# facebookresearch/wmar

Hardware: AMD Instinct MI355X
Metric: watermarked images/sec at 256x256 (16x16 tok), batch 64; detector p-value delta vs ref (higher is better)
Workload: dtype f32; 1 GPU; Taming cin_transformer (48L x 1536d x 24h, V=16384) + VQGAN f16/16384, 256x256, batch 64 per GPU, greenlist watermark delta=2 gamma=0.25 h=1 (linear/stratifiedrand), T=1 top-k 250 top-p 0.92; sample -> decode -> re-encode -> detect; random-init weights; batch_per_gpu=64, decode_loop=hipGraph replay, backend=nccl

## Files before the change

wmar_amd/csrc/decoder_kernels.h:

```cpp
#pragma once
#include <cstdint>

#include "sampler.h"
#include "bx_split.h"

namespace wmar {

using f32x16 = __attribute__((ext_vector_type(16))) float;
using f32x4 = __attribute__((ext_vector_type(4))) float;

__device__ __forceinline__ float4 ld_nt(const float4* p) {
    f32x4 v = __builtin_nontemporal_load((const f32x4*)p);
    return make_float4(v.x, v.y, v.z, v.w);
}

__device__ __forceinline__ void st_out(float4* p, const float4 v) {
#ifndef WMAR_PLAIN_STORES
    const f32x4 q = {v.x, v.y, v.z, v.w};
    asm volatile("global_store_dwordx4 %0, %1, off sc1\n\ts_nop 1" :: "v"(p), "v"(q) : "memory");
#else
    *p = v;
#endif
}
using f32x2 = __attribute__((ext_vector_type(2))) float;
// ... 677 lines not shown

constexpr int QX_CK = 4;
#ifndef QX_ABL
#define QX_ABL 0
#endif
#define WMAR_QX_SYNC() if (!(QX_ABL & 2)) __syncthreads();
#ifndef QX_SPLIT
#define QX_SPLIT 2
#endif

struct QkvxArgs {
    const float4* Wp;
    const float4* x_in;
    float4* x_out;
    const float4* slabs;
    long long slab_stride;
    int n_hi;
    const float* bias;
    double* stats;
    float4* out;
    long long out_stride;
    int KB, NT, S, cap;
    int nkeep;
    unsigned long long* trace;
    unsigned long long* trace_chunks;
};

template <int MTW, int S_IN>
__global__ __launch_bounds__(512) void k_qkvx(QkvxArgs a) {
    __shared__ __attribute__((aligned(16))) float4 xs[2][QX_CK][MTW][64];
    __shared__ double red[4][MTW][64][2];
    const int lane = threadIdx.x & 63;
    const int w = __builtin_amdgcn_readfirstlane(threadIdx.x >> 6);
    const int half = lane >> 5;
    const int G = a.NT >> 2;
    const int j = (int)(blockIdx.x & 7) * a.cap + (int)(blockIdx.x >> 3);
    if (j >= G * a.S) return;
    const int s = j / G, g = j - s * G;
    const int kb0 = (int)((unsigned)s * (unsigned)a.KB / (unsigned)a.S);
    const int kb1 = (int)((unsigned)(s + 1) * (unsigned)a.KB / (unsigned)a.S);
    const int nkb = kb1 - kb0, nch = (nkb + QX_CK - 1) / QX_CK;
    const bool keeper = g == 0;

    if (w >= 4) {
        const int sw = w - 4;
        double sum[MTW], sq[MTW];
// ... 191 lines not shown
static int launch_qkvx(const QkvxArgs& q, int MT, int S_in, hipStream_t st) {
    if (MT == 1) return launch_qkvx_mt<1>(q, S_in, st);
    if (MT == 2) return launch_qkvx_mt<2>(q, S_in, st);
    set_error("qkvx: %d row tiles unsupported", MT);
    return WMAR_EINVAL;
}

static __global__ void k_pack_bx(const float* __restrict__ W, const float* __restrict__ gamma, float4* __restrict__ Wq, int N, int K,
                                      int tile_off) {
    const long long idx = (long long)blockIdx.x * blockDim.x + threadIdx.x;
    const int KU = K / 16;
    if (idx >= (long long)(N / 32) * KU * 128) return;
    const int lane = (int)(idx & 63), hf = (int)((idx >> 6) & 1);
    const long long r = idx >> 7;
    const int ku = (int)(r % KU), tile = (int)(r / KU);
    const int k = ku * 16 + 8 * (lane >> 5) + 4 * hf;
    const float* p = W + (long long)(tile * 32 + (lane & 31)) * K + k;
    float4 v = make_float4(p[0], p[1], p[2], p[3]);
    if (gamma) { v.x *= gamma[k]; v.y *= gamma[k + 1]; v.z *= gamma[k + 2]; v.w *= gamma[k + 3]; }
    Wq[idx + (long long)tile_off * KU * 128] = v;
}

constexpr int QX_TR_STRIDE = 36;
template <int S_IN>
__global__ __launch_bounds__(512) void k_qkvx_bx(QkvxArgs a) {
    constexpr int MTW = 2;
    __shared__ __attribute__((aligned(16))) u32x4 xq[2][2][MTW][3][64];
    __shared__ __attribute__((aligned(16))) float tr_s[4][32 * QX_TR_STRIDE];
    __shared__ double red[4][MTW][64][2];
    const int lane = threadIdx.x & 63;
    const int w = __builtin_amdgcn_readfirstlane(threadIdx.x >> 6);
    const int half = lane >> 5;
    const int G = a.NT >> 2;
    const int j = (int)(blockIdx.x & 7) * a.cap + (int)(blockIdx.x >> 3);
    if (j >= G * a.S) return;
    const int s = j / G, g = j - s * G;
    const int KU = a.KB >> 1;
    const int kb0 = 2 * (int)((unsigned)s * (unsigned)KU / (unsigned)a.S);
    const int kb1 = 2 * (int)((unsigned)(s + 1) * (unsigned)KU / (unsigned)a.S);
    const int nkb = kb1 - kb0, nch = (nkb + QX_CK - 1) / QX_CK;
    const bool keeper = g < a.nkeep;

    if (w >= 4) {
        const int sw = w - 4;
        double sum[MTW], sq[MTW];
#pragma unroll
        for (int i = 0; i < MTW; ++i) { sum[i] = 0.0; sq[i] = 0.0; }
        float4 xvA[MTW], bbA, slA[S_IN > 0 ? S_IN : 1][MTW];
        float4 xvB[MTW], bbB, slB[S_IN > 0 ? S_IN : 1][MTW];
        int skbA = 0, skbB = 0;
#define WMAR_QX_ISSUE(XV, BB, SL, SKB, C)                                                              \
    {                                                                                                   \
        SKB = kb0 + (C) * QX_CK + sw;                                                                   \
        const int kk = SKB < kb1 ? SKB : kb1 - 1;                                                       \
        const long long idx = (long long)kk * MTW * 64 + lane;                                          \
        _Pragma("unroll") for (int i = 0; i < MTW; ++i) XV[i] = a.x_in[idx + i * 64];                   \
        if (S_IN > 0) {                                                                                 \
            BB = *(const float4*)(a.bias + kk * 8 + 4 * half);                                          \
            _Pragma("unroll") for (int si = 0; si < S_IN; ++si)                                         \
                _Pragma("unroll") for (int i = 0; i < MTW; ++i)                                         \
                    SL[si][i] = a.slabs[(long long)si * a.slab_stride + idx + i * 64];                  \
        }                                                                                               \
    }
#define WMAR_QX_FINISH(XV, BB, SL, SKB, BUF, CIDX)                                                     \
    if (SKB < kb1) {                                                                                    \
        const bool short_tile = a.n_hi > 0 && (SKB >> 2) >= a.n_hi;                                     \
        _Pragma("unroll") for (int i = 0; i < MTW; ++i) {                                               \
            float4 r = XV[i];                                                                           \
            if (S_IN > 0) {                                                                             \
                float4 t = SL[0][i];                                                                    \
                _Pragma("unroll") for (int si = 1; si < S_IN; ++si)                                     \
                    if (!(si == S_IN - 1 && short_tile)) {                                              \
                        t.x += SL[si][i].x; t.y += SL[si][i].y; t.z += SL[si][i].z; t.w += SL[si][i].w; \
                    }                                                                                   \
                r = make_float4(r.x + (BB.x + t.x), r.y + (BB.y + t.y), r.z + (BB.z + t.z), r.w + (BB.w + t.w)); \
            }                                                                                           \
            unsigned h0, m0, l0, h1, m1, l1;                                                            \
            bx_split2(r.x, r.y, h0, m0, l0);                                                            \
            bx_split2(r.z, r.w, h1, m1, l1);                                                            \
            u32x2* d = (u32x2*)&xq[BUF][sw >> 1][i][0][(lane & 31) + 32 * (sw & 1)] + half;             \
            d[0] = u32x2{h0, h1}; d[128] = u32x2{m0, m1}; d[256] = u32x2{l0, l1};                       \
            if (keeper && (CIDX) % a.nkeep == g) {                                                      \
                a.x_out[((long long)SKB * MTW + i) * 64 + lane] = r;                                    \
                sum[i] += (double)r.x + (double)r.y + (double)r.z + (double)r.w;                        \
                sq[i] += sq4_f64(r);                        \
            }                                                                                           \
        }                                                                                               \
    }
        WMAR_QX_ISSUE(xvA, bbA, slA, skbA, 0)
        WMAR_QX_ISSUE(xvB, bbB, slB, skbB, 1)
        __builtin_amdgcn_sched_barrier(0);
        WMAR_QX_FINISH(xvA, bbA, slA, skbA, 0, 0)
        __builtin_amdgcn_sched_barrier(0);
        WMAR_QX_ISSUE(xvA, bbA, slA, skbA, 2)
        __builtin_amdgcn_sched_barrier(0);
        __syncthreads();
        for (int c = 0; c + 1 < nch; c += 2) {
            WMAR_QX_FINISH(xvB, bbB, slB, skbB, 1, c + 1)
            __builtin_amdgcn_sched_barrier(0);
            WMAR_QX_ISSUE(xvB, bbB, slB, skbB, c + 3)
            __builtin_amdgcn_sched_barrier(0);
            __syncthreads();
            if (c + 2 >= nch) break;
            WMAR_QX_FINISH(xvA, bbA, slA, skbA, 0, c + 2)
            __builtin_amdgcn_sched_barrier(0);
            WMAR_QX_ISSUE(xvA, bbA, slA, skbA, c + 4)
            __builtin_amdgcn_sched_barrier(0);
            __syncthreads();
        }
#undef WMAR_QX_ISSUE
#undef WMAR_QX_FINISH
        if (keeper) {
#pragma unroll
            for (int i = 0; i < MTW; ++i) {
                red[sw][i][lane][0] = sum[i]; red[sw][i][lane][1] = sq[i];
            }
            __syncthreads();
            const int t = threadIdx.x - 256;
            if (t < 32 * MTW) {
                const int i = t >> 5, r = t & 31;
                double ts = 0, tss = 0;
                for (int ww = 0; ww < 4; ++ww) { ts += red[ww][i][r][0] + red[ww][i][r + 32][0]; tss += red[ww][i][r][1] + red[ww][i][r + 32][1]; }
                double* o = a.stats + ((long long)(s * a.nkeep + g) * (MTW * 32) + i * 32 + r) * 2;
                o[0] = ts; o[1] = tss;
            }
        }
        return;
    }

    WMAR_ST_BEGIN
    const int nt = g * 4 + w;
    f32x16 acc[MTW];
#pragma unroll
// ... 67 lines not shown
#undef WMAR_QX_STEP
#pragma unroll
    for (int i = 0; i < MTW; ++i) {
        float* T = &tr_s[w][0];
#pragma unroll
        for (int q4 = 0; q4 < 4; ++q4)
            *(float4*)(T + (lane & 31) * QX_TR_STRIDE + 8 * q4 + 4 * half) =
                make_float4(acc[i][q4 * 4 + 0], acc[i][q4 * 4 + 1], acc[i][q4 * 4 + 2], acc[i][q4 * 4 + 3]);
        __builtin_amdgcn_wave_barrier();
        asm volatile("s_waitcnt lgkmcnt(0)" ::: "memory");
#pragma unroll
        for (int it = 0; it < 4; ++it) {
            const int row = (lane >> 3) + 8 * it, cg = lane & 7;
            const float4 v = *(const float4*)(T + row * QX_TR_STRIDE + 4 * cg);
            st_out(a.out + (long long)s * a.out_stride + ((long long)(32 * i + row) * (a.NT * 32) + nt * 32 + 4 * cg) / 4, v);
        }
        __builtin_amdgcn_wave_barrier();
        asm volatile("s_waitcnt lgkmcnt(0)" ::: "memory");
    }
    WMAR_ST_END(a.trace, j)
    if (keeper) __syncthreads();
}

static int launch_qkvx_bx(const QkvxArgs& q, int S_in, hipStream_t st) {
    const dim3 grid((unsigned)(8 * q.cap));
    switch (S_in) {
#define WMAR_QX_CASE(N) case N: hipLaunchKernelGGL((k_qkvx_bx<N>), grid, dim3(512), 0, st, q); break;
        WMAR_QX_CASE(0) WMAR_QX_CASE(1) WMAR_QX_CASE(2) WMAR_QX_CASE(3) WMAR_QX_CASE(4)
        WMAR_QX_CASE(5) WMAR_QX_CASE(6) WMAR_QX_CASE(7) WMAR_QX_CASE(8)
#undef WMAR_QX_CASE
        default: set_error("qkvx_bx: bad slab count %d", S_in); return WMAR_EINVAL;
    }
    return launch_status("k_qkvx_bx");
}


struct BxArgs {
    const float4* Wq;
    const u32x4* Xq;
    float4* out;
    long long slab_stride;
    int KU;
    int S;
    const float* bias;
    u32x4* outq;
    int rowmajor;
    int N;
};

#define WMAR_BX_MFMA(A, B, C) C = __builtin_amdgcn_mfma_f32_32x32x16_bf16(A, B, C, 0, 0, 0)

template <int NT, int PER, int MTW = 2, bool GELU = false, int NW = 4, bool XF = false>
__global__ __launch_bounds__(NW * 64) void k_bx(BxArgs a) {
    constexpr int XR = XF ? 2 * MTW : 3 * MTW;
    constexpr int ROWS = NT * 4 * MTW;
    __shared__ __attribute__((aligned(16))) float4 red[NW][ROWS][64];
// ... 831 lines not shown
```

wmar_amd/csrc/gpt.hip:

```cpp
#include <cstdint>
#include <map>
#include <string>
#include <vector>

#include "decoder_host.h"
#include "decode_small.h"
#include "decode_persist.h"


using namespace wmar;

struct LayerW {
    float4 *wqkv, *wproj, *wfc1, *wfc2;
    float4* wfc1x16 = nullptr;
    float2* wfc1x8 = nullptr;
    float4* wqkvx_bx = nullptr;
    float4* wproj_bx = nullptr;
    float *bqkv, *bproj, *bfc1, *bfc2, *cqkv, *cfc1;
};

struct SmallW {
    float *wqkv = nullptr, *bqkv = nullptr, *wproj = nullptr, *bproj = nullptr, *wfc1 = nullptr, *bfc1 = nullptr, *wfc2 = nullptr, *bfc2 = nullptr;
    float *ln1w = nullptr, *ln1b = nullptr, *ln2w = nullptr, *ln2b = nullptr;
};
// ... 33 lines not shown
    unsigned long long graph_key[12] = {0};
    bool pending = false;
    void drop_graph() {
        if (pending && ev1) (void)hipEventSynchronize(ev1);
        pending = false;
        for (int i = 0; i < N_PHASE; ++i) {
            if (exec[i]) (void)hipGraphExecDestroy(exec[i]);
            if (graph[i]) (void)hipGraphDestroy(graph[i]);
            exec[i] = nullptr; graph[i] = nullptr;
        }
    }
    int att_t1 = 1 << 30, att_t2 = 1 << 30;
    bool att_user = false;
    int att_phase(int kv, int64_t B) const {
        if (!att_user && B * H < 512) return kv <= 128 ? 1 : 2;
        return kv <= att_t1 ? 0 : (kv <= att_t2 ? 1 : 2);
    }
    static int phase_waves(int ph) { return ph == 0 ? 1 : (ph == 1 ? 2 : 4); }
    int timing = 0;
    bool no_bx_qkv = false, no_bx_proj = false;
    unsigned* xsync = nullptr;
    bool xcd_ok = false;
    bool no_xr = false;
    int inject_fail = 0;
    int fallbacks = 0;
    unsigned long long* dbg_sums = nullptr; int dbg_slot = 0;
    unsigned long long* stamps = nullptr;
    unsigned long long* stamp_slot(int l, int role) const {
        return stamps ? stamps + ((long long)(l * 5 + role) * WMAR_STAMP_UNITS) * 8 : nullptr;
    }
    bool no_bx = false;
    int force_s[3] = {0, 0, 0};
    double step_ms = 0.0;
    struct Span { int cls; hipEvent_t a, b; };
    std::vector<Span> spans;
    std::vector<hipEvent_t> ev_pool;
    size_t ev_used = 0;
    bool span_on = false;
    double cls_us[WMAR_T_NCLASS] = {0};
    int64_t cls_calls[WMAR_T_NCLASS] = {0};
    hipEvent_t next_event() {
        if (ev_used == ev_pool.size()) {
            hipEvent_t e = nullptr;
            (void)hipEventCreate(&e);
            ev_pool.push_back(e);
        }
// ... 99 lines not shown
        }
        const int NTq = 3 * D / 32;
        if (g->force_s[0] <= 0 && NTq % 4 == 0 && MT <= 2 && S_fc2 + (fc2_hi > 0 ? 1 : 0) <= MAX_SLABS) {
            const int G = NTq / 4;
            int S = 256 / G;
            if (S > QKV_SLABS_MAX) S = QKV_SLABS_MAX;
            if (S > KBD / QX_CK) S = KBD / QX_CK;
            if (S >= 1) S_qx = S;
        }
        proj_bx = MT == 2 && g->yq && g->layers[0].wproj_bx && !g->no_bx && !g->no_bx_proj && g->force_s[1] <= 0;
        if (proj_bx) S_proj = D / BX_KSLICE;
        proj_xr = proj_bx && g->xcd_ok && !g->no_xr && S_proj == 4 && (D / 32) % 8 == 0 && (D / 32 / 8) * S_proj <= 32 && (D / 32 / 8) % 2 == 0;
        nch_ln2 = proj_xr ? 16 : nch;
    }
    void dbg(const void* p, long long bytes) {
#ifdef WMAR_DEV_KNOBS
        if (!g->dbg_sums || g->dbg_slot >= 4096) return;
        hipLaunchKernelGGL(k_dbg_sum, dim3(512), dim3(256), 0, st, (const uint32_t*)p, bytes / 4, g->dbg_sums + g->dbg_slot++);
#else
        (void)p; (void)bytes;
#endif
    }
    bool qkv_bx() const { return S_qx > 0 && MT == 2 && g->layers[0].wqkvx_bx && !g->no_bx && !g->no_bx_qkv; }
    bool fc1_x() const { return MT == 2 && g->layers[0].wfc1x16 && nch_ln2 <= 16; }
    int qx_nkeep() const { const int G = 3 * D / 128; return G >= 4 && S_qx * 4 <= STAT_CHUNKS_MAX ? 4 : 1; }
    static bool head_narrow() { static int v = -1; if (v < 0) v = getenv("WMAR_HEAD_NARROW") ? 1 : 0; return v != 0; }
    int split_for(int NT, int KB) const { return pick_split(MT % 2 == 0 ? NT * (MT / 2) : NT * MT, KB, 4); }
    GemmArgs base() const {
        GemmArgs a{};
        a.MT = MT; a.B = (int)B; a.stats = g->stats; a.n_chunks = nch; a.K = D;
        a.pos_dev = g->pos_dev; a.D = D; a.H = g->H; a.hd = g->hd; a.Tmax = g->Tmax;
        return a;
    }
    SgArgs sg_base() const {
        SgArgs a{};
        a.pos_dev = g->pos_dev; a.D = D; a.H = g->H; a.Tmax = g->Tmax;
        return a;
    }
    int embed() {
        if (small) {
            SeArgs e{g->tok_emb, g->pos_emb, g->xs, io.tok, io.tok_stride, io.tok_use_pos, g->pos_dev, D};
            g->span_begin(WMAR_T_EMBED, st);
            hipLaunchKernelGGL(k_sembed, dim3((unsigned)((D / 4 + 255) / 256), (unsigned)B), dim3(256), 0, st, e);
            g->span_end(st);
            return launch_status("k_sembed");
        }
// ... 3 lines not shown
        g->span_end(st);
        return launch_status("k_resid_stats<embed>");
    }
    int resid(const float* bias, int S, int n_hi = 0) {
        r.x = xcur;
        r.S = S + (n_hi > 0 ? 1 : 0); r.bias = bias; r.n_hi = n_hi;
        g->span_begin(WMAR_T_RESID, st);
        int rc = launch_resid(r, nch * MT, st);
        g->span_end(st);
        return rc;
    }
    int qkvx(int l, const float* prev_bias) {
        QkvxArgs q{};
        const LayerW& w = g->layers[l];
        float4* xout = (xcur == g->x) ? g->x2 : g->x;
        q.Wp = w.wqkv; q.x_in = xcur; q.x_out = xout;
        q.slabs = g->slabs; q.slab_stride = act;
        const int S_in = prev_bias ? S_fc2 + (fc2_hi > 0 ? 1 : 0) : 0;
        q.n_hi = prev_bias ? fc2_hi : 0; q.bias = prev_bias;
        q.stats = g->stats_q; q.out = g->qkv_slabs; q.out_stride = 3 * act;
        q.KB = KBD; q.NT = 3 * D / 32; q.S = S_qx;
        q.cap = ((q.NT / 4) * q.S + 7) / 8;
        q.nkeep = qx_nkeep();
        q.trace = g->stamp_slot(l, 0);
        g->span_begin(WMAR_T_QKV, st);
        int rc;
        if (qkv_bx()) { q.Wp = w.wqkvx_bx; rc = launch_qkvx_bx(q, S_in, st); }
        else rc = launch_qkvx(q, MT, S_in, st);
        g->span_end(st);
        xcur = xout;
        return rc;
    }
    int qkv_small(int l) {
        const SmallW& w = g->sw[l];
        const long long lstride = (long long)g->Bmax * g->H * g->Tmax * g->hd;
        SgArgs a = sg_base();
        a.W = w.wqkv; a.bias = g->layers[l].bqkv; a.c1 = g->layers[l].cqkv; a.x = g->xs; a.gamma = w.ln1w; a.out = g->qs;
        a.kcache = g->kcache + l * lstride; a.vcache = g->vcache + l * lstride; a.N = 3 * D; a.K = D;
        g->span_begin(WMAR_T_QKV, st);
        const int rc = launch_sgemv<3, 3, SG_QKV>(a, (int)B, st);
        g->span_end(st);
        return rc;
    }
    int qkv(int l) {
        GemmArgs a = base();
        const LayerW& w = g->layers[l];
        a.Wp = w.wqkv; a.Xp = xcur; a.KB = KBD; a.NT = 3 * D / 32;
        a.out_packed = g->qkv_slabs; a.slab_stride = 3 * act;
        int S = 1;
        g->span_begin(WMAR_T_QKV, st);
// ... 183 lines not shown
        a.arena = g->sw_arena; a.L = g->L; a.tok_emb = g->tok_emb; a.pos_emb = g->pos_emb; a.whead = g->whead_rm; a.lnfw = g->lnfw; a.lnfb = g->lnfb;
        a.tok = io.tok; a.tok_stride = io.tok_stride; a.tok_use_pos = io.tok_use_pos;
        a.xs = g->xs; a.ys = g->ys; a.hs = g->hs; a.qs = g->qs; a.kcache = g->kcache; a.vcache = g->vcache;
        a.lstride = (long long)g->Bmax * g->H * g->Tmax * g->hd; a.logits = io.logits; a.V = g->V; a.pos_dev = g->pos_dev;
        a.D = g->D; a.H = g->H; a.Tmax = g->Tmax; a.bar = g->ss_bar;
        g->span_begin(WMAR_T_QKV, st);
        rc = launch_sstep(a, (int)B, st);
        g->span_end(st);
        g->ps_enqueued = true;
        return rc;
    }
    if ((rc = p.embed())) return rc;
    if (p.small) {
        for (int l = 0; l < g->L; ++l) {
            if ((rc = p.qkv_small(l))) return rc;
            if ((rc = p.attn(l))) return rc;
            if ((rc = p.proj(l))) return rc;
            if ((rc = p.fc1(l))) return rc;
            if ((rc = p.fc2(l))) return rc;
        }
        return p.head();
    }
    p.dbg(p.xcur, actb); p.dbg(g->stats, p.nch * Mpad * 16);
    for (int l = 0; l < g->L; ++l) {
        if (p.S_qx > 0) {
            if ((rc = p.qkvx(l, l > 0 ? g->layers[l - 1].bfc2 : nullptr))) return rc;
            p.dbg(p.xcur, actb); p.dbg(g->stats_q, p.S_qx * Mpad * 16); p.dbg(g->qkv_slabs, p.S_qx * 3 * actb);
        } else {
            if (l > 0 && (rc = p.resid(g->layers[l - 1].bfc2, p.S_fc2, p.fc2_hi))) return rc;
            if ((rc = p.qkv(l))) return rc;
            p.dbg(p.xcur, actb); p.dbg(g->stats, p.nch * Mpad * 16); p.dbg(g->qkv_slabs, 3 * actb);
        }
        if ((rc = p.attn(l))) return rc;
        if (p.proj_bx) p.dbg(g->yq, (long long)p.D / 16 * 2 * 3 * 64 * 16); else p.dbg(g->y, actb);
        {
            const long long lstride = (long long)g->Bmax * g->H * g->Tmax * g->hd;
            p.dbg(g->kcache + l * lstride, lstride * 4); p.dbg(g->vcache + l * lstride, lstride * 4);
        }
        if ((rc = p.proj(l))) return rc;
        p.dbg(g->slabs, p.S_proj * actb);
        if (!p.proj_xr && (rc = p.resid(g->layers[l].bproj, p.S_proj))) return rc;
        p.dbg(p.xcur, actb); p.dbg(g->stats, p.nch_ln2 * Mpad * 16);
        if ((rc = p.fc1(l))) return rc;
        p.dbg(g->hbuf, 4 * actb);
        if ((rc = p.fc2(l))) return rc;
        p.dbg(g->slabs, p.S_fc2 * actb);
// ... 180 lines not shown
                g->persist_ok = ok;
            }
        }
    }
    const size_t Mpad = (size_t)g->MTmax * 32;
    TRY(g->alloc(&g->x, Mpad * D / 4));
    TRY(g->alloc(&g->x2, Mpad * D / 4));
    TRY(g->alloc(&g->y, Mpad * D / 4));
    TRY(g->alloc(&g->hbuf, Mpad * 4 * D / 4));
    TRY(g->alloc(&g->slabs, (size_t)MAX_SLABS * Mpad * D / 4));
    TRY(g->alloc(&g->qkv_slabs, (size_t)MAX_SLABS * Mpad * 3 * D / 4));
    if (g->MTmax >= 2 && D % BX_KSLICE == 0) TRY(g->alloc(&g->yq, (size_t)D / 16 * 2 * 3 * 64));
    TRY(g->alloc(&g->qbuf, Mpad * D));
    TRY(g->alloc(&g->stats, (size_t)STAT_CHUNKS_MAX * Mpad * 2));
    TRY(g->alloc(&g->stats_q, (size_t)QKV_SLABS_MAX * 4 * Mpad * 2));
    const size_t kv = (size_t)L * g->Bmax * H * g->Tmax * hd;
    TRY(g->alloc(&g->kcache, kv));
    TRY(g->alloc(&g->vcache, kv));
    TRY(g->alloc(&g->logits, (size_t)g->Bmax * V));
    TRY(g->alloc(&g->scratch, (size_t)g->Bmax * V));
    TRY(g->alloc(&g->past, (size_t)g->Bmax * (g->Tmax + 1)));
    TRY(g->alloc(&g->pos_dev, 4));
    TRY(g->alloc(&g->xsync, 8 * 64 + 64));
    g->step_dev = g->pos_dev + 1;
    if (rc == WMAR_OK) {
        hipError_t e = hipMemsetAsync(g->x, 0, Mpad * D * 4, st);
        if (e == hipSuccess) e = hipMemsetAsync(g->x2, 0, Mpad * D * 4, st);
        if (e == hipSuccess) e = hipMemsetAsync(g->kcache, 0, kv * 4, st);
        if (e == hipSuccess) e = hipMemsetAsync(g->vcache, 0, kv * 4, st);
        if (e == hipSuccess) e = hipMemsetAsync(g->hbuf, 0, Mpad * 4 * D * 4, st);
        if (e == hipSuccess) e = hipMemsetAsync(g->past, 0, (size_t)g->Bmax * (g->Tmax + 1) * 8, st);
        if (e == hipSuccess) e = hipMemsetAsync(g->y, 0, Mpad * D * 4, st);
        if (e == hipSuccess) e = hipMemsetAsync(g->qbuf, 0, Mpad * D * 4, st);
        if (e == hipSuccess && g->yq) e = hipMemsetAsync(g->yq, 0, (size_t)D / 16 * 2 * 3 * 64 * 16, st);
        if (e == hipSuccess) e = hipMemsetAsync(g->xsync, 0, (8 * 64 + 64) * 4, st);
        if (e == hipSuccess) e = hipStreamCreateWithFlags(&g->cap_stream, hipStreamNonBlocking);
        if (e == hipSuccess) e = hipEventCreate(&g->ev0);
        if (e == hipSuccess) e = hipEventCreate(&g->ev1);
        if (e == hipSuccess) e = hipStreamSynchronize(st);
        if (e != hipSuccess) { set_error("gpt_create: %s", hipGetErrorString(e)); rc = WMAR_EHIP; }
    }
#undef TRY
    if (rc == WMAR_OK && g->MTmax >= 2 && g->yq) {
        g->no_xr = getenv("WMAR_NO_XR") != nullptr;
        unsigned* tmp = nullptr;
        bool ok = hipMalloc(&tmp, 192 * 4) == hipSuccess;
        for (int rep = 0; rep < 3 && ok; ++rep) {
            unsigned h[192];
            hipLaunchKernelGGL(k_xcc_probe, dim3(192), dim3(256), 0, st, tmp);
            ok = hipMemcpyAsync(h, tmp, sizeof h, hipMemcpyDeviceToHost, st) == hipSuccess && hipStreamSynchronize(st) == hipSuccess;
            unsigned seen = 0;
            for (int b = 0; b < 192 && ok; ++b) ok = h[b] == h[b & 7] && h[b] < 16;
            for (int x = 0; x < 8 && ok; ++x) { ok = !(seen & (1u << h[x])); seen |= 1u << h[x]; }
        }
        if (tmp) (void)hipFree(tmp);
        int nb = 0, dev = 0, cus = 0;
        const bool xr4 = getenv("WMAR_XR_NW4") != nullptr;
        if (ok) ok = (xr4 ? hipOccupancyMaxActiveBlocksPerMultiprocessor(&nb, k_bx_xr<BX_PER, 4>, 256, 0)
                          : hipOccupancyMaxActiveBlocksPerMultiprocessor(&nb, k_bx_xr<BX_PER / 2, 4, 8>, 512, 0)) == hipSuccess && hipGetDevice(&dev) == hipSuccess &&
                     hipDeviceGetAttribute(&cus, hipDeviceAttributeMultiprocessorCount, dev) == hipSuccess &&
                     (long long)nb * cus >= (long long)(D / 32) * 4;
        g->xcd_ok = ok;
        { const char* e = getenv("WMAR_INJECT_SYNC_FAIL"); g->inject_fail = (e && atoi(e) > 0) ? 1 : 0; }
    }
    if (rc != WMAR_OK) { delete g; return rc; }
    *out = g;
    return WMAR_OK;
}

static int gpt_persist_failed(wmar_gpt* g, hipStream_t st) {
    if (!g->ss_bar || !g->persist_ok || !g->ps_enqueued) return 0;
    g->ps_enqueued = false;
    unsigned f = 0;
    WMAR_HIP_CHECK(hipMemcpyAsync(&f, g->ss_bar + 8 * 64 + 64, 4, hipMemcpyDeviceToHost, st));
    WMAR_HIP_CHECK(hipStreamSynchronize(st));
    if (!f) return 0;
    g->drop_graph();
    WMAR_HIP_CHECK(hipMemsetAsync(g->ss_bar, 0, SS_BAR_WORDS * 4, st));
    g->persist_ok = false;
    g->fallbacks += 1;
    fprintf(stderr, "wmar_amd: the persistent decode step (k_sstep) gave up waiting at its device-wide barrier; this engine continues on the "
                    "five-launch small-batch plan (the call is re-run; wmar_gpt_plan_info reports barrier_fallbacks)\n");
    return 1;
}
static int gpt_sync_failed(wmar_gpt* g, hipStream_t st) {
    if (const int pf = gpt_persist_failed(g, st)) return pf;
    if (!g->xsync || !g->xcd_ok || g->no_xr || !g->xr_enqueued) return 0;
    g->xr_enqueued = false;
    unsigned f[2] = {0, 0};
    WMAR_HIP_CHECK(hipMemcpyAsync(f, g->xsync + 8 * 64, 8, hipMemcpyDeviceToHost, st));
    WMAR_HIP_CHECK(hipStreamSynchronize(st));
    if (!f[0] && !f[1]) return 0;
    g->drop_graph();
    WMAR_HIP_CHECK(hipMemsetAsync(g->xsync, 0, (8 * 64 + 64) * 4, st));
    g->xcd_ok = false;
    g->fallbacks += 1;
    fprintf(stderr, "wmar_amd: the fused projection launch (k_bx_xr) %s; this engine continues on the two-launch path (the call is re-run; "
                    "wmar_gpt_plan_info reports barrier_fallbacks)\n", f[0] ? "found a workgroup on a foreign XCD" : "gave up waiting at its XCD-local barrier");
    return 1;
}
static int gpt_inject(wmar_gpt* g, hipStream_t st) {
    if (!g->inject_fail || !g->xcd_ok) return WMAR_OK;
    g->inject_fail = 0;
    hipLaunchKernelGGL(k_set_int, dim3(1), dim3(1), 0, st, (int*)(g->xsync + 8 * 64 + 1), 1);
    return launch_status("k_set_int");
}
int wmar_gpt_check(wmar_gpt* g, void* stream) {
    WMAR_REQUIRE(g, "gpt_check: null argument");
    const int f = gpt_sync_failed(g, (hipStream_t)stream);
    if (f < 0) return f;
    if (f > 0) {
        set_error("gpt: the XCD-local barrier of the fused projection launch gave up or found a block on a foreign XCD: the launches since "
                  "the last check are invalid (the engine continues on the two-launch path)");
        return WMAR_EHIP;
    }
    return WMAR_OK;
}

void wmar_gpt_destroy(wmar_gpt* g) { delete g; }
int64_t wmar_gpt_device_bytes(const wmar_gpt* g) { return g ? g->bytes : 0; }

// ... 14 lines not shown
    }
    set_error("decode_step: the in-launch barrier flag is up on the two-launch path");
    return WMAR_EHIP;
}

int wmar_gpt_profile_role(wmar_gpt* g, int32_t role, int64_t B, int32_t kv_len, int32_t iters, void* stream,
                          double* avg_us) {
    WMAR_REQUIRE(g && avg_us && iters > 0, "profile_role: bad argument");
    WMAR_REQUIRE(B >= 1 && B <= g->Bmax, "profile_role: batch outside 1..%d", g->Bmax);
    WMAR_REQUIRE(kv_len >= 1 && kv_len <= g->Tmax, "profile_role: kv_len outside 1..%d", g->Tmax);
    hipStream_t st = (hipStream_t)stream;
    hipLaunchKernelGGL(k_set_int, dim3(1), dim3(1), 0, st, g->pos_dev, (int)kv_len - 1);
    StepIO io{g->past, (long long)g->Tmax + 1, 0, g->logits};
    g->att_nw = wmar_gpt::phase_waves(g->att_phase(kv_len, B));
    StepPlan p(g, B, io, st);
    int ncycle = g->L;
#ifdef WMAR_DEV_KNOBS
    { const char* pl = getenv("WMAR_PROFILE_LAYERS"); if (pl && atoi(pl) > 0) ncycle = std::min(atoi(pl), g->L); }
#endif
    auto one = [&](int it) -> int {
        const int l = it % ncycle;
        switch (role) {
            case WMAR_T_EMBED: return p.embed();
            case WMAR_T_QKV: if (p.small) return p.qkv_small(l); p.xcur = g->x; return p.S_qx > 0 ? p.qkvx(l, g->layers[l].bfc2) : p.qkv(l);
            case WMAR_T_ATTN: return p.attn(l);
            case WMAR_T_PROJ: return p.proj(l);
            case WMAR_T_RESID: if (p.small) { set_error("profile_role: the small-batch path has no residual launch"); return WMAR_EINVAL; } return p.resid(g->layers[l].bproj, p.S_proj);
            case WMAR_T_FC1: return p.fc1(l);
            case WMAR_T_FC2: return p.fc2(l);
            case WMAR_T_HEAD: return p.head();
            default: set_error("profile_role: unknown role %d", role); return WMAR_EINVAL;
        }
    };
    const bool was = g->span_on;
    g->span_on = false;
    int rc = WMAR_OK;
    for (int i = 0; i < 3 && rc == WMAR_OK; ++i) rc = one(i);
    if (rc == WMAR_OK && hipEventRecord(g->ev0, st) != hipSuccess) rc = WMAR_EHIP;
    for (int i = 0; i < iters && rc == WMAR_OK; ++i) rc = one(i + 3);
    if (rc == WMAR_OK && hipEventRecord(g->ev1, st) != hipSuccess) rc = WMAR_EHIP;
    g->span_on = was;
    if (rc) return rc;
    WMAR_HIP_CHECK(hipEventSynchronize(g->ev1));
    float ms = 0.f;
    WMAR_HIP_CHECK(hipEventElapsedTime(&ms, g->ev0, g->ev1));
    *avg_us = (double)ms * 1000.0 / iters;
    return WMAR_OK;
// ... 3 lines not shown
    WMAR_REQUIRE(g && buf && buf_len > 0, "plan_info: null argument");
    WMAR_REQUIRE(B >= 1 && B <= g->Bmax, "plan_info: batch outside 1..%d", g->Bmax);
    StepIO io{g->past, (long long)g->Tmax + 1, 0, g->logits};
    StepPlan p(g, B, io, nullptr);
    if (p.persist) {
        const int n = snprintf(buf, (size_t)buf_len,
                               "qkv=k_sstep phase (the arithmetic of k_sgemv<QKV>, weights streamed across the barriers);attn=k_sstep phase;proj=k_sstep phase;resid=none;"
                               "resid_launches_per_step=0;fc1=k_sstep phase;fc2=k_sstep phase;head=k_sstep phase;barrier_fallbacks=%d;"
                               "path=persistent step: one launch, %d device-wide barriers (decode_persist.h)", g->fallbacks, 5 * g->L + 1);
        WMAR_REQUIRE(n > 0 && n < buf_len, "plan_info: buffer of %lld bytes too small", (long long)buf_len);
        return WMAR_OK;
    }
    if (p.small) {
        const int n = snprintf(buf, (size_t)buf_len,
                               "qkv=k_sgemv<QKV> (row-major weight stream, LN1 + bias + cache append inside, %d columns per workgroup);"
                               "attn=k_sattn (4 waves per (sequence, head));proj=k_sgemv<PROJ> (residual added in place);resid=none;"
                               "resid_launches_per_step=0;fc1=k_sgemv<FC1> (LN2 + bias + GELU inside);fc2=k_sgemv<FC2> (8 K segments, residual added in place);"
                               "head=k_sgemv<HEAD> (ln_f inside);barrier_fallbacks=%d;path=small-batch streaming (decode_small.h)",
                               sg_cols_wg<3, 3, SG_QKV>(), g->fallbacks);
        WMAR_REQUIRE(n > 0 && n < buf_len, "plan_info: buffer of %lld bytes too small", (long long)buf_len);
        return WMAR_OK;
    }
    const LayerW& w = g->layers[0];
    char qkv[96], proj[160], fc1[96], fc2[96];
    const int S_in = p.S_fc2 + (p.fc2_hi > 0 ? 1 : 0);
    (void)w;
    if (p.qkv_bx()) snprintf(qkv, sizeof qkv, "k_qkvx_bx<%d> (bf16 pipe, %d K slices)", S_in, p.S_qx);
    else if (p.S_qx > 0) snprintf(qkv, sizeof qkv, "k_qkvx<%d,%d> (fp32 MFMA, %d K slices)", p.MT, S_in, p.S_qx);
    else snprintf(qkv, sizeof qkv, "k_gemm<EPI_PACKED> (fp32 MFMA, %d K slices) after k_resid_stats", p.S_qkv);
    if (p.proj_xr) snprintf(proj, sizeof proj, "k_bx_xr<%d,4> (bf16 pipe, 4 K slices + XCD-local reduction: residual fold and LN2 statistics inside)", BX_PER);
    else if (p.proj_bx) snprintf(proj, sizeof proj, "k_bx<1,%d> (bf16 pipe, %d K slices)", BX_PER, p.S_proj);
    else snprintf(proj, sizeof proj, "k_gemm<EPI_PACKED> (fp32 MFMA, %d K slices)", p.S_proj);
    if (p.fc1_x()) snprintf(fc1, sizeof fc1, "k_fc1x (fp32 MFMA, 24-column tiles, whole K)");
    else snprintf(fc1, sizeof fc1, "k_gemm<EPI_GELU,LN> (fp32 MFMA, whole K)");
    snprintf(fc2, sizeof fc2, "k_gemm<EPI_PACKED> (fp32 MFMA, %d%s K slices)", p.S_fc2, p.fc2_hi > 0 ? "/+1" : "");
    char attn[96];
    const int w0 = wmar_gpt::phase_waves(g->att_phase(1, B)), w1 = wmar_gpt::phase_waves(g->att_phase(g->Tmax / 2, B)),
              w2 = wmar_gpt::phase_waves(g->att_phase(g->Tmax, B));
    if (w0 == w1 && w1 == w2) snprintf(attn, sizeof attn, "k_attn_decode<%d,%d>", g->hd, w1);
    else snprintf(attn, sizeof attn, "k_attn_decode<%d,%d> (%d / %d / %d waves at 1 / %d / %d cached rows)", g->hd, w1, w0, w1, w2, g->Tmax / 2, g->Tmax);
    const int n = snprintf(buf, (size_t)buf_len, "qkv=%s;attn=%s;proj=%s;resid=k_resid_stats;resid_launches_per_step=%d;fc1=%s;fc2=%s;head=k_gemm<EPI_LOGITS,LN> (fp32 MFMA);barrier_fallbacks=%d",
                           qkv, attn, proj, p.proj_xr ? 1 : g->L + 1, fc1, fc2, g->fallbacks);
    WMAR_REQUIRE(n > 0 && n < buf_len, "plan_info: buffer of %lld bytes too small", (long long)buf_len);
    return WMAR_OK;
}

#ifdef WMAR_STAMPS
int wmar_gpt_debug_stamps(wmar_gpt* g, unsigned long long* out, long long n_u64) {
    WMAR_REQUIRE(g && g->stamps && out, "debug_stamps: not enabled (WMAR_STAMPS=1 at creation of a -DWMAR_STAMPS build)");
    const long long n = (long long)g->L * 5 * WMAR_STAMP_UNITS * 8;
// ... 197 lines not shown
```

Measured before the change: 59.23 images/s.

## Fold QKV residual once per K slice with cross-workgroup hand-off

Adds a k_qkvx_bx_xf variant. In it, the workgroups sharing a K slice split the residual fold (x + bias + fc2 slab partials) among themselves and write the folded x once. Each then signals an atomic counter, and the others poll it before reading the folded x instead of re-summing the slabs themselves. This removes redundant slab reads and adds across the column groups. In exchange it adds spin-wait synchronisation, per-layer counters reset each step, and a timeout fallback path.

Result: no change. 59.82 images/s (median of 6 runs) (+1.0%).

```diff
diff --git a/wmar_amd/csrc/decoder_kernels.h b/wmar_amd/csrc/decoder_kernels.h
--- a/wmar_amd/csrc/decoder_kernels.h
+++ b/wmar_amd/csrc/decoder_kernels.h
@@ -723,6 +723,8 @@
     long long out_stride;
     int KB, NT, S, cap;
     int nkeep;
+    unsigned* xf_cnt;
+    unsigned* xf_fail;
     unsigned long long* trace;
     unsigned long long* trace_chunks;
 };
@@ -960,12 +962,15 @@
 }
 
 constexpr int QX_TR_STRIDE = 36;
-template <int S_IN>
-__global__ __launch_bounds__(512) void k_qkvx_bx(QkvxArgs a) {
+constexpr int QX_XF_MAX_POLLS = 1 << 15;
+
+template <int S_IN, bool XF>
+__device__ __forceinline__ void qkvx_bx_body(const QkvxArgs& a) {
     constexpr int MTW = 2;
     __shared__ __attribute__((aligned(16))) u32x4 xq[2][2][MTW][3][64];
     __shared__ __attribute__((aligned(16))) float tr_s[4][32 * QX_TR_STRIDE];
     __shared__ double red[4][MTW][64][2];
+    __shared__ unsigned xf_ready;
     const int lane = threadIdx.x & 63;
     const int w = __builtin_amdgcn_readfirstlane(threadIdx.x >> 6);
     const int half = lane >> 5;
@@ -987,31 +992,37 @@
         float4 xvA[MTW], bbA, slA[S_IN > 0 ? S_IN : 1][MTW];
         float4 xvB[MTW], bbB, slB[S_IN > 0 ? S_IN : 1][MTW];
         int skbA = 0, skbB = 0;
-#define WMAR_QX_ISSUE(XV, BB, SL, SKB, C)                                                              \
+#define WMAR_QX_ISSUE(XV, BB, SL, SKB, C, SRC, FOLD)                                                   \
     {                                                                                                   \
         SKB = kb0 + (C) * QX_CK + sw;                                                                   \
         const int kk = SKB < kb1 ? SKB : kb1 - 1;                                                       \
         const long long idx = (long long)kk * MTW * 64 + lane;                                          \
-        _Pragma("unroll") for (int i = 0; i < MTW; ++i) XV[i] = a.x_in[idx + i * 64];                   \
-        if (S_IN > 0) {                                                                                 \
+        _Pragma("unroll") for (int i = 0; i < MTW; ++i) XV[i] = (SRC)[idx + i * 64];                    \
+        if ((FOLD) && S_IN > 0) {                                                                       \
             BB = *(const float4*)(a.bias + kk * 8 + 4 * half);                                          \
             _Pragma("unroll") for (int si = 0; si < S_IN; ++si)                                         \
                 _Pragma("unroll") for (int i = 0; i < MTW; ++i)                                         \
                     SL[si][i] = a.slabs[(long long)si * a.slab_stride + idx + i * 64];                  \
         }                                                                                               \
     }
-#define WMAR_QX_FINISH(XV, BB, SL, SKB, BUF, CIDX)                                                     \
+#define WMAR_QX_FOLD(R, XV, BB, SL, SHORT)                                                             \
+    {                                                                                                   \
+        float4 t = SL[0];                                                                               \
+        _Pragma("unroll") for (int si = 1; si < S_IN; ++si)                                             \
+            if (!(si == S_IN - 1 && (SHORT))) {                                                         \
+                t.x += SL[si].x; t.y += SL[si].y; t.z += SL[si].z; t.w += SL[si].w;                     \
+            }                                                                                           \
+        R = make_float4(XV.x + (BB.x + t.x), XV.y + (BB.y + t.y), XV.z + (BB.z + t.z), XV.w + (BB.w + t.w)); \
+    }
+#define WMAR_QX_FINISH(XV, BB, SL, SKB, BUF, CIDX, FOLD)                                               \
     if (SKB < kb1) {                                                                                    \
         const bool short_tile = a.n_hi > 0 && (SKB >> 2) >= a.n_hi;                                     \
         _Pragma("unroll") for (int i = 0; i < MTW; ++i) {                                               \
             float4 r = XV[i];                                                                           \
-            if (S_IN > 0) {                                                                             \
-                float4 t = SL[0][i];                                                                    \
-                _Pragma("unroll") for (int si = 1; si < S_IN; ++si)                                     \
-                    if (!(si == S_IN - 1 && short_tile)) {                                              \
-                        t.x += SL[si][i].x; t.y += SL[si][i].y; t.z += SL[si][i].z; t.w += SL[si][i].w; \
-                    }                                                                                   \
-                r = make_float4(r.x + (BB.x + t.x), r.y + (BB.y + t.y), r.z + (BB.z + t.z), r.w + (BB.w + t.w)); \
+            if ((FOLD) && S_IN > 0) {                                                                   \
+                float4 sl_[S_IN > 0 ? S_IN : 1];                                                        \
+                _Pragma("unroll") for (int si = 0; si < S_IN; ++si) sl_[si] = SL[si][i];                \
+                WMAR_QX_FOLD(r, XV[i], BB, sl_, short_tile)                                             \
             }                                                                                           \
             unsigned h0, m0, l0, h1, m1, l1;                                                            \
             bx_split2(r.x, r.y, h0, m0, l0);                                                            \
@@ -1019,34 +1030,121 @@
             u32x2* d = (u32x2*)&xq[BUF][sw >> 1][i][0][(lane & 31) + 32 * (sw & 1)] + half;             \
             d[0] = u32x2{h0, h1}; d[128] = u32x2{m0, m1}; d[256] = u32x2{l0, l1};                       \
             if (keeper && (CIDX) % a.nkeep == g) {                                                      \
-                a.x_out[((long long)SKB * MTW + i) * 64 + lane] = r;                                    \
+                if (!XF) a.x_out[((long long)SKB * MTW + i) * 64 + lane] = r;                           \
                 sum[i] += (double)r.x + (double)r.y + (double)r.z + (double)r.w;                        \
                 sq[i] += sq4_f64(r);                        \
             }                                                                                           \
         }                                                                                               \
     }
-        WMAR_QX_ISSUE(xvA, bbA, slA, skbA, 0)
-        WMAR_QX_ISSUE(xvB, bbB, slB, skbB, 1)
-        __builtin_amdgcn_sched_barrier(0);
-        WMAR_QX_FINISH(xvA, bbA, slA, skbA, 0, 0)
-        __builtin_amdgcn_sched_barrier(0);
-        WMAR_QX_ISSUE(xvA, bbA, slA, skbA, 2)
-        __builtin_amdgcn_sched_barrier(0);
-        __syncthreads();
-        for (int c = 0; c + 1 < nch; c += 2) {
-            WMAR_QX_FINISH(xvB, bbB, slB, skbB, 1, c + 1)
+        if constexpr (!XF) {
+            WMAR_QX_ISSUE(xvA, bbA, slA, skbA, 0, a.x_in, true)
+            WMAR_QX_ISSUE(xvB, bbB, slB, skbB, 1, a.x_in, true)
             __builtin_amdgcn_sched_barrier(0);
-            WMAR_QX_ISSUE(xvB, bbB, slB, skbB, c + 3)
+            WMAR_QX_FINISH(xvA, bbA, slA, skbA, 0, 0, true)
+            __builtin_amdgcn_sched_barrier(0);
+            WMAR_QX_ISSUE(xvA, bbA, slA, skbA, 2, a.x_in, true)
             __builtin_amdgcn_sched_barrier(0);
             __syncthreads();
-            if (c + 2 >= nch) break;
-            WMAR_QX_FINISH(xvA, bbA, slA, skbA, 0, c + 2)
+            for (int c = 0; c + 1 < nch; c += 2) {
+                WMAR_QX_FINISH(xvB, bbB, slB, skbB, 1, c + 1, true)
+                __builtin_amdgcn_sched_barrier(0);
+                WMAR_QX_ISSUE(xvB, bbB, slB, skbB, c + 3, a.x_in, true)
+                __builtin_amdgcn_sched_barrier(0);
+                __syncthreads();
+                if (c + 2 >= nch) break;
+                WMAR_QX_FINISH(xvA, bbA, slA, skbA, 0, c + 2, true)
+                __builtin_amdgcn_sched_barrier(0);
+                WMAR_QX_ISSUE(xvA, bbA, slA, skbA, c + 4, a.x_in, true)
+                __builtin_amdgcn_sched_barrier(0);
+                __syncthreads();
+            }
+        } else {
+            const int U = MTW * nkb;
+            const int v = sw * G + g;
+            float4 ux, ub, us[S_IN > 0 ? S_IN : 1];
+            int ukb = 0, ui = 0;
+#define WMAR_QX_UNIT_LOAD(U_)                                                                          \
+    {                                                                                                   \
+        ukb = kb0 + (U_) / MTW; ui = (U_) % MTW;                                                        \
+        const long long uidx = ((long long)ukb * MTW + ui) * 64 + lane;                                 \
+        ux = a.x_in[uidx];                                                                              \
+        ub = *(const float4*)(a.bias + ukb * 8 + 4 * half);                                             \
+        _Pragma("unroll") for (int si = 0; si < S_IN; ++si) us[si] = a.slabs[(long long)si * a.slab_stride + uidx]; \
+    }
+#define WMAR_QX_UNIT_STORE()                                                                           \
+    {                                                                                                   \
+        float4 r;                                                                                       \
+        WMAR_QX_FOLD(r, ux, ub, us, a.n_hi > 0 && (ukb >> 2) >= a.n_hi)                                 \
+        st_out(a.x_out + ((long long)ukb * MTW + ui) * 64 + lane, r);                                   \
+    }
+            if (v < U) WMAR_QX_UNIT_LOAD(v)
+            WMAR_QX_ISSUE(xvA, bbA, slA, skbA, 0, a.x_in, true)
+            WMAR_QX_ISSUE(xvB, bbB, slB, skbB, 1, a.x_in, true)
             __builtin_amdgcn_sched_barrier(0);
-            WMAR_QX_ISSUE(xvA, bbA, slA, skbA, c + 4)
+            unsigned nu = 0;
+            if (v < U) {
+                WMAR_QX_UNIT_STORE()
+                nu = 1;
+                for (int u = v + 4 * G; u < U; u += 4 * G) {
+                    WMAR_QX_UNIT_LOAD(u)
+                    WMAR_QX_UNIT_STORE()
+                    ++nu;
+                }
+            }
+#undef WMAR_QX_UNIT_LOAD
+#undef WMAR_QX_UNIT_STORE
             __builtin_amdgcn_sched_barrier(0);
+            WMAR_QX_FINISH(xvA, bbA, slA, skbA, 0, 0, true)
+            __builtin_amdgcn_sched_barrier(0);
+            if (sw == 0 && lane == 0) xf_ready = 0u;
             __syncthreads();
+            if (nu) {
+                asm volatile("s_waitcnt vmcnt(0)" ::: "memory");
+                if (lane == 0) __hip_atomic_fetch_add(a.xf_cnt + s * 32, nu, __ATOMIC_RELAXED, __HIP_MEMORY_SCOPE_AGENT);
+            }
+            WMAR_QX_FINISH(xvB, bbB, slB, skbB, 1, 1, true)
+            __builtin_amdgcn_sched_barrier(0);
+            if (1 < nch) __syncthreads();
+            if (2 < nch) {
+                if (sw == 0 && lane == 0) {
+                    const unsigned* cnt = a.xf_cnt + s * 32;
+                    unsigned spins = 0;
+                    bool dead = __hip_atomic_load(a.xf_fail + 1, __ATOMIC_RELAXED, __HIP_MEMORY_SCOPE_AGENT) != 0u;
+                    while (!dead && __hip_atomic_load(cnt, __ATOMIC_RELAXED, __HIP_MEMORY_SCOPE_AGENT) < (unsigned)U) {
+                        __builtin_amdgcn_s_sleep(1);
+                        ++spins;
+                        if ((spins & 255) == 0) dead = __hip_atomic_load(a.xf_fail + 1, __ATOMIC_RELAXED, __HIP_MEMORY_SCOPE_AGENT) != 0u;
+                        if (spins > QX_XF_MAX_POLLS) { __hip_atomic_store(a.xf_fail + 1, 1u, __ATOMIC_RELAXED, __HIP_MEMORY_SCOPE_AGENT); break; }
+                    }
+                }
+                if (sw == 0) {
+                    __builtin_amdgcn_fence(__ATOMIC_ACQUIRE, "agent");
+                    asm volatile("s_waitcnt vmcnt(0)" ::: "memory");
+                    if (lane == 0) __hip_atomic_store(&xf_ready, 1u, __ATOMIC_RELAXED, __HIP_MEMORY_SCOPE_WORKGROUP);
+                } else {
+                    while (__hip_atomic_load(&xf_ready, __ATOMIC_RELAXED, __HIP_MEMORY_SCOPE_WORKGROUP) == 0u) __builtin_amdgcn_s_sleep(1);
+                }
+                __builtin_amdgcn_fence(__ATOMIC_ACQUIRE, "workgroup");
+                WMAR_QX_ISSUE(xvA, bbA, slA, skbA, 2, a.x_out, false)
+                WMAR_QX_ISSUE(xvB, bbB, slB, skbB, 3, a.x_out, false)
+                __builtin_amdgcn_sched_barrier(0);
+            }
+            for (int c = 1; c + 1 < nch; c += 2) {
+                WMAR_QX_FINISH(xvA, bbA, slA, skbA, 0, c + 1, false)
+                __builtin_amdgcn_sched_barrier(0);
+                WMAR_QX_ISSUE(xvA, bbA, slA, skbA, c + 3, a.x_out, false)
+                __builtin_amdgcn_sched_barrier(0);
+                __syncthreads();
+                if (c + 2 >= nch) break;
+                WMAR_QX_FINISH(xvB, bbB, slB, skbB, 1, c + 2, false)
+                __builtin_amdgcn_sched_barrier(0);
+                WMAR_QX_ISSUE(xvB, bbB, slB, skbB, c + 4, a.x_out, false)
+                __builtin_amdgcn_sched_barrier(0);
+                __syncthreads();
+            }
         }
 #undef WMAR_QX_ISSUE
+#undef WMAR_QX_FOLD
 #undef WMAR_QX_FINISH
         if (keeper) {
 #pragma unroll
@@ -1160,6 +1258,11 @@
     if (keeper) __syncthreads();
 }
 
+template <int S_IN>
+__global__ __launch_bounds__(512) void k_qkvx_bx(QkvxArgs a) { qkvx_bx_body<S_IN, false>(a); }
+template <int S_IN>
+__global__ __launch_bounds__(512) void k_qkvx_bx_xf(QkvxArgs a) { qkvx_bx_body<S_IN, true>(a); }
+
 static int launch_qkvx_bx(const QkvxArgs& q, int S_in, hipStream_t st) {
     const dim3 grid((unsigned)(8 * q.cap));
     switch (S_in) {
@@ -1170,6 +1273,17 @@
         default: set_error("qkvx_bx: bad slab count %d", S_in); return WMAR_EINVAL;
     }
     return launch_status("k_qkvx_bx");
+}
+static int launch_qkvx_bx_xf(const QkvxArgs& q, int S_in, hipStream_t st) {
+    const dim3 grid((unsigned)(8 * q.cap));
+    switch (S_in) {
+#define WMAR_QX_CASE(N) case N: hipLaunchKernelGGL((k_qkvx_bx_xf<N>), grid, dim3(512), 0, st, q); break;
+        WMAR_QX_CASE(1) WMAR_QX_CASE(2) WMAR_QX_CASE(3) WMAR_QX_CASE(4)
+        WMAR_QX_CASE(5) WMAR_QX_CASE(6) WMAR_QX_CASE(7) WMAR_QX_CASE(8)
+#undef WMAR_QX_CASE
+        default: set_error("qkvx_bx_xf: bad slab count %d", S_in); return WMAR_EINVAL;
+    }
+    return launch_status("k_qkvx_bx_xf");
 }
 
 
diff --git a/wmar_amd/csrc/gpt.hip b/wmar_amd/csrc/gpt.hip
--- a/wmar_amd/csrc/gpt.hip
+++ b/wmar_amd/csrc/gpt.hip
@@ -79,6 +79,9 @@
     unsigned* xsync = nullptr;
     bool xcd_ok = false;
     bool no_xr = false;
+    unsigned* qxsync = nullptr;
+    bool qx_xf_ok = false;
+    bool no_qx_xcd = false;
     int inject_fail = 0;
     int fallbacks = 0;
     unsigned long long* dbg_sums = nullptr; int dbg_slot = 0;
@@ -224,6 +227,8 @@
 #endif
     }
     bool qkv_bx() const { return S_qx > 0 && MT == 2 && g->layers[0].wqkvx_bx && !g->no_bx && !g->no_bx_qkv; }
+    bool qkv_xf() const { return qkv_bx() && g->qxsync && g->qx_xf_ok && g->xcd_ok && !g->no_xr && !g->no_qx_xcd; }
+    long long qx_sync_bytes() const { return (long long)g->L * 8 * 32 * 4; }
     bool fc1_x() const { return MT == 2 && g->layers[0].wfc1x16 && nch_ln2 <= 16; }
     int qx_nkeep() const { const int G = 3 * D / 128; return G >= 4 && S_qx * 4 <= STAT_CHUNKS_MAX ? 4 : 1; }
     static bool head_narrow() { static int v = -1; if (v < 0) v = getenv("WMAR_HEAD_NARROW") ? 1 : 0; return v != 0; }
@@ -273,10 +278,15 @@
         q.KB = KBD; q.NT = 3 * D / 32; q.S = S_qx;
         q.cap = ((q.NT / 4) * q.S + 7) / 8;
         q.nkeep = qx_nkeep();
+        q.xf_cnt = g->qxsync + (long long)l * 8 * 32; q.xf_fail = g->xsync + 8 * 64;
         q.trace = g->stamp_slot(l, 0);
         g->span_begin(WMAR_T_QKV, st);
         int rc;
-        if (qkv_bx()) { q.Wp = w.wqkvx_bx; rc = launch_qkvx_bx(q, S_in, st); }
+        if (qkv_bx() && S_in > 0 && qkv_xf()) {
+            q.Wp = w.wqkvx_bx; rc = launch_qkvx_bx_xf(q, S_in, st);
+            g->xr_enqueued = true;
+        }
+        else if (qkv_bx()) { q.Wp = w.wqkvx_bx; rc = launch_qkvx_bx(q, S_in, st); }
         else rc = launch_qkvx(q, MT, S_in, st);
         g->span_end(st);
         xcur = xout;
@@ -506,6 +516,7 @@
         return p.head();
     }
     p.dbg(p.xcur, actb); p.dbg(g->stats, p.nch * Mpad * 16);
+    if (p.S_qx > 0 && p.qkv_xf() && hipMemsetAsync(g->qxsync, 0, (size_t)p.qx_sync_bytes(), st) != hipSuccess) return WMAR_EHIP;
     for (int l = 0; l < g->L; ++l) {
         if (p.S_qx > 0) {
             if ((rc = p.qkvx(l, l > 0 ? g->layers[l - 1].bfc2 : nullptr))) return rc;
@@ -732,6 +743,7 @@
     TRY(g->alloc(&g->past, (size_t)g->Bmax * (g->Tmax + 1)));
     TRY(g->alloc(&g->pos_dev, 4));
     TRY(g->alloc(&g->xsync, 8 * 64 + 64));
+    TRY(g->alloc(&g->qxsync, (size_t)L * 8 * 32));
     g->step_dev = g->pos_dev + 1;
     if (rc == WMAR_OK) {
         hipError_t e = hipMemsetAsync(g->x, 0, Mpad * D * 4, st);
@@ -744,6 +756,7 @@
         if (e == hipSuccess) e = hipMemsetAsync(g->qbuf, 0, Mpad * D * 4, st);
         if (e == hipSuccess && g->yq) e = hipMemsetAsync(g->yq, 0, (size_t)D / 16 * 2 * 3 * 64 * 16, st);
         if (e == hipSuccess) e = hipMemsetAsync(g->xsync, 0, (8 * 64 + 64) * 4, st);
+        if (e == hipSuccess) e = hipMemsetAsync(g->qxsync, 0, (size_t)L * 8 * 32 * 4, st);
         if (e == hipSuccess) e = hipStreamCreateWithFlags(&g->cap_stream, hipStreamNonBlocking);
         if (e == hipSuccess) e = hipEventCreate(&g->ev0);
         if (e == hipSuccess) e = hipEventCreate(&g->ev1);
@@ -772,6 +785,19 @@
                      (long long)nb * cus >= (long long)(D / 32) * 4;
         g->xcd_ok = ok;
         { const char* e = getenv("WMAR_INJECT_SYNC_FAIL"); g->inject_fail = (e && atoi(e) > 0) ? 1 : 0; }
+        g->no_qx_xcd = getenv("WMAR_NO_QX_XCD") != nullptr;
+        {
+            const int G = 3 * D / 128;
+            int S = G > 0 ? 256 / G : 0;
+            if (S > QKV_SLABS_MAX) S = QKV_SLABS_MAX;
+            if (S > D / 8 / QX_CK) S = D / 8 / QX_CK;
+            const int grid = 8 * ((G * S + 7) / 8);
+            int nq = 0, qdev = 0, qcus = 0;
+            g->qx_xf_ok = (3 * D) % 128 == 0 && S >= 1 &&
+                          hipOccupancyMaxActiveBlocksPerMultiprocessor(&nq, k_qkvx_bx_xf<1>, 512, 0) == hipSuccess && nq >= 1 &&
+                          hipGetDevice(&qdev) == hipSuccess && hipDeviceGetAttribute(&qcus, hipDeviceAttributeMultiprocessorCount, qdev) == hipSuccess &&
+                          qcus >= grid;
+        }
     }
     if (rc != WMAR_OK) { delete g; return rc; }
     *out = g;
@@ -805,8 +831,9 @@
     WMAR_HIP_CHECK(hipMemsetAsync(g->xsync, 0, (8 * 64 + 64) * 4, st));
     g->xcd_ok = false;
     g->fallbacks += 1;
-    fprintf(stderr, "wmar_amd: the fused projection launch (k_bx_xr) %s; this engine continues on the two-launch path (the call is re-run; "
-                    "wmar_gpt_plan_info reports barrier_fallbacks)\n", f[0] ? "found a workgroup on a foreign XCD" : "gave up waiting at its XCD-local barrier");
+    fprintf(stderr, "wmar_amd: the fused projection launch (k_bx_xr) or the QKV launch's fold hand-off (k_qkvx_bx_xf) %s; this engine continues "
+                    "on the two-launch path and k_qkvx_bx (the call is re-run; wmar_gpt_plan_info reports barrier_fallbacks)\n",
+            f[0] ? "found a workgroup on a foreign XCD" : "gave up waiting");
     return 1;
 }
 static int gpt_inject(wmar_gpt* g, hipStream_t st) {
@@ -867,7 +894,11 @@
         const int l = it % ncycle;
         switch (role) {
             case WMAR_T_EMBED: return p.embed();
-            case WMAR_T_QKV: if (p.small) return p.qkv_small(l); p.xcur = g->x; return p.S_qx > 0 ? p.qkvx(l, g->layers[l].bfc2) : p.qkv(l);
+            case WMAR_T_QKV:
+                if (p.small) return p.qkv_small(l);
+                p.xcur = g->x;
+                if (p.S_qx > 0 && p.qkv_xf() && l == 0 && hipMemsetAsync(g->qxsync, 0, (size_t)p.qx_sync_bytes(), st) != hipSuccess) return WMAR_EHIP;
+                return p.S_qx > 0 ? p.qkvx(l, g->layers[l].bfc2) : p.qkv(l);
             case WMAR_T_ATTN: return p.attn(l);
             case WMAR_T_PROJ: return p.proj(l);
             case WMAR_T_RESID: if (p.small) { set_error("profile_role: the small-batch path has no residual launch"); return WMAR_EINVAL; } return p.resid(g->layers[l].bproj, p.S_proj);
@@ -917,10 +948,11 @@
         return WMAR_OK;
     }
     const LayerW& w = g->layers[0];
-    char qkv[96], proj[160], fc1[96], fc2[96];
+    char qkv[160], proj[160], fc1[96], fc2[96];
     const int S_in = p.S_fc2 + (p.fc2_hi > 0 ? 1 : 0);
     (void)w;
-    if (p.qkv_bx()) snprintf(qkv, sizeof qkv, "k_qkvx_bx<%d> (bf16 pipe, %d K slices)", S_in, p.S_qx);
+    if (p.qkv_xf()) snprintf(qkv, sizeof qkv, "k_qkvx_bx_xf<%d> (bf16 pipe, %d K slices, residual fold once per K slice, layer 0 k_qkvx_bx<0>)", S_in, p.S_qx);
+    else if (p.qkv_bx()) snprintf(qkv, sizeof qkv, "k_qkvx_bx<%d> (bf16 pipe, %d K slices)", S_in, p.S_qx);
     else if (p.S_qx > 0) snprintf(qkv, sizeof qkv, "k_qkvx<%d,%d> (fp32 MFMA, %d K slices)", p.MT, S_in, p.S_qx);
     else snprintf(qkv, sizeof qkv, "k_gemm<EPI_PACKED> (fp32 MFMA, %d K slices) after k_resid_stats", p.S_qkv);
     if (p.proj_xr) snprintf(proj, sizeof proj, "k_bx_xr<%d,4> (bf16 pipe, 4 K slices + XCD-local reduction: residual fold and LN2 statistics inside)", BX_PER);
```
